# tontinton/dbeel

Measured on NVIDIA H100. Metric: compaction throughput MB/s (input bytes) at 1/2/4/8 H100 vs CPU shards, higher is better.
Workload: dtype u8

## Files before the change

dbeel_b200/csrc/dbeel_compact.cu:

```cuda
#include <cuda_runtime.h>
#include <math.h>
#include <stdint.h>
#include <stdio.h>
#include <stdlib.h>
#include <string.h>

#include <algorithm>
#include <atomic>
#include <deque>
#include <memory>
#include <new>
#include <thread>
#include <string>
#include <vector>

#include "../../include/dbeel_compact.h"
#include "kernels.cuh"
#include "merge_final.cuh"
#include "gather_async.cuh"
#include "gather_fb.cuh"
#include "gather_h.cuh"
#include "lookup.cuh"
#include "lookup_stream.cuh"
#include "route.cuh"
#include "scan.cuh"
#include "wal.cuh"
#include "host/scan_plan.h"
#include "host/stream_pump.h"

using namespace dbeel;

namespace {

constexpr uint64_t kAlign = 256;
inline uint64_t align_up(uint64_t v, uint64_t a) { return (v + a - 1) / a * a; }

enum { EV_START = 0, EV_EXTRACT, EV_MERGE, EV_RESOLVE, EV_GATHER, EV_H2D0, EV_H2D1, EV_D2H0, EV_D2H1, EV_COUNT };

}

struct dbeel_engine {
    int device = 0;
    cudaStream_t stream = nullptr;
    cudaEvent_t ev[EV_COUNT] = {};
    uint8_t *ws = nullptr;
    uint64_t ws_cap = 0;
    uint8_t *stage_in = nullptr, *stage_out = nullptr;
    uint64_t stage_in_cap = 0, stage_out_cap = 0;
    uint8_t *stage_in2 = nullptr, *stage_out2 = nullptr, *bloom_dev = nullptr;
    uint64_t stage_in2_cap = 0, stage_out2_cap = 0, bloom_dev_cap = 0;
    cudaStream_t s_h2d = nullptr, s_d2h = nullptr;
    cudaEvent_t ev_h2d[2] = {}, ev_comp[2] = {}, ev_d2h[2] = {};
    int pipeline = 1;
    uint64_t pipeline_min_bytes = 64ull << 20;
    uint64_t partition_bytes = 256ull << 20;
    int partition_taper = 1;
    uint8_t *ring_in = nullptr, *ring_out = nullptr, *pin_index = nullptr, *pin_bloom = nullptr;
    uint64_t ring_in_cap = 0, ring_out_cap = 0, pin_index_cap = 0, pin_bloom_cap = 0;
    int stream_ring = 3;
    uint8_t *wal_ws = nullptr;
    uint64_t wal_ws_cap = 0;
    uint8_t *route_ws = nullptr;
    uint64_t route_ws_cap = 0;
    uint8_t *pin = nullptr;
    uint8_t *pin_dev = nullptr;
    uint64_t pin_cap = 0;
    dbeel_stats stats = {};
    std::string err;
    bool busy = false;
    std::thread worker;
    std::atomic<int> async_state{0};
    int async_status = 0;
    std::vector<dbeel_run> async_runs;
    dbeel_compact_opts async_opts = {};
    uint8_t async_seed[32] = {};
    int sm_count = 0;
    int merge_variant = 1;
    int narrow_loads = 1;
    int gather_variant = 11;
    int fused_emit = 0;
    int bloom_side = 0;
    cudaStream_t s_side = nullptr;
    cudaEvent_t ev_fork = nullptr, ev_join = nullptr;
    int fused_final = 1;
    int fin_ctas_per_sm = 0;
    int pdl = 0;
    int stage_events = 1;
    int extract_persist = 6;
    int bloom_in_extract = 0;
};

namespace {

int fail(dbeel_engine *e, int code, const char *what, cudaError_t ce = cudaSuccess) {
    char buf[512];
    if (ce != cudaSuccess)
        snprintf(buf, sizeof buf, "%s: %s (%s)", what, cudaGetErrorName(ce), cudaGetErrorString(ce));
    else
        snprintf(buf, sizeof buf, "%s", what);
    if (e) e->err = buf;
    return code;
}

#define CU(call)                                                            \
    do {                                                                    \
        cudaError_t ce_ = (call);                                           \
        if (ce_ != cudaSuccess) return fail(e, DBEEL_ERR_CUDA, #call, ce_); \
    } while (0)

int ensure_device(dbeel_engine *e, uint8_t **buf, uint64_t *cap, uint64_t need) {
    if (need <= *cap) return DBEEL_OK;
    if (*buf) { cudaFree(*buf); *buf = nullptr; *cap = 0; }
    uint64_t want = align_up(need + need / 8, 1 << 20);
    cudaError_t ce = cudaMalloc(reinterpret_cast<void **>(buf), want);
    if (ce != cudaSuccess) {
        cudaGetLastError();
        want = align_up(need, 1 << 20);
        ce = cudaMalloc(reinterpret_cast<void **>(buf), want);
    }
    if (ce != cudaSuccess) { cudaGetLastError(); return fail(e, DBEEL_ERR_NOMEM, "cudaMalloc(workspace)", ce); }
    *cap = want;
    return DBEEL_OK;
}

int ensure_pinned(dbeel_engine *e, uint64_t need) {
    if (need <= e->pin_cap) return DBEEL_OK;
    if (e->pin) cudaFreeHost(e->pin);
    e->pin = nullptr;
    e->pin_dev = nullptr;
    e->pin_cap = 0;
    cudaError_t ce = cudaHostAlloc(reinterpret_cast<void **>(&e->pin), need, cudaHostAllocMapped);
    if (ce != cudaSuccess) { cudaGetLastError(); return fail(e, DBEEL_ERR_NOMEM, "cudaHostAlloc", ce); }
    ce = cudaHostGetDevicePointer(reinterpret_cast<void **>(&e->pin_dev), e->pin, 0);
    if (ce != cudaSuccess) { cudaGetLastError(); return fail(e, DBEEL_ERR_CUDA, "cudaHostGetDevicePointer", ce); }
    e->pin_cap = need;
    return DBEEL_OK;
}

int ensure_host(dbeel_engine *e, uint8_t **buf, uint64_t *cap, uint64_t need) {
    if (need <= *cap) return DBEEL_OK;
    if (*buf) { cudaFreeHost(*buf); *buf = nullptr; *cap = 0; }
    const uint64_t want = align_up(need + need / 8, 1 << 20);
    cudaError_t ce = cudaHostAlloc(reinterpret_cast<void **>(buf), want, cudaHostAllocDefault);
    if (ce != cudaSuccess) { cudaGetLastError(); *buf = nullptr; return fail(e, DBEEL_ERR_NOMEM, "cudaHostAlloc(stream ring)", ce); }
    *cap = want;
    return DBEEL_OK;
}

int stream_threads() {
    static const int n = [] {
        if (const char *v = getenv("DBEEL_IO_THREADS")) return std::max(1, atoi(v));
        const unsigned hw = std::thread::hardware_concurrency();
        return (int)std::min(8u, std::max(2u, hw / 8));
    }();
    return n;
}

template <class F>
int parallel_pieces(size_t n, F fn) {
    std::atomic<size_t> next{0};
    std::atomic<int> err{0};
    auto work = [&]() {
        for (size_t k = next.fetch_add(1); k < n && !err.load(); k = next.fetch_add(1)) {
            const int rc = fn(k);
            if (rc) { int z = 0; err.compare_exchange_strong(z, rc); }
        }
    };
    const int nt = (int)std::min<size_t>((size_t)stream_threads(), n);
// ... 274 lines not shown
            if (!f || fread(seed, 1, 32, f) != 32) {
                if (f) fclose(f);
                return fail(e, DBEEL_ERR_INVALID_ARG, "no entropy source for the bloom seed");
            }
            fclose(f);
        }
        p.bloom.words = reinterpret_cast<uint32_t *>(static_cast<uint8_t *>(out->bloom) + 8);
        p.bloom.bits = sh.bloom_bits;
        p.bloom.bits_magic = (uint64_t)((((unsigned __int128)1) << 64) / sh.bloom_bits);
        p.bloom.k_num = sh.bloom_k;
        for (int i = 0; i < 4; i++) memcpy(&p.bloom.sip[i], seed + 8 * i, 8);
    }
    if (extra) {
        p.sparse_offsets = extra->sparse_offsets ? 1 : 0;
        p.out_offset_base = extra->out_offset_base;
        if (extra->external_bloom) p.bloom = extra->bloom;
    }

    cudaStream_t s = e->stream;
    uint32_t launches = 0;
    if (record_start) CU(cudaEventRecord(e->ev[EV_START], s));
    launch_k(e, k_copy_words, (uint32_t)((header_bytes / 4 + 255) / 256), 256, 0, s, reinterpret_cast<uint32_t *>(ws),
             reinterpret_cast<const uint32_t *>(e->pin_dev), (uint32_t)(header_bytes / 4));
    launches++;
    if (sh.bloom_file) CU(cudaMemsetAsync(out->bloom, 0, sh.bloom_file, s));
    if (scan_bytes) CU(cudaMemsetAsync(ws + o_scan, 0, scan_bytes, s));

    const uint32_t g256 = (N + 255) / 256;
    const uint32_t gext = (N + 256 * kExtractEPT - 1) / (256 * kExtractEPT);
    auto launch_extract = [&](uint32_t grid, int mode) {
        if (ref_reader && hash_early) launch_k(e, k_extract<true, true, true>, grid, 256, 0, s, p, mode);
        else if (ref_reader) launch_k(e, k_extract<true, true, false>, grid, 256, 0, s, p, mode);
        else if (hash_early) launch_k(e, k_extract<true, false, true>, grid, 256, 0, s, p, mode);
        else if (e->narrow_loads && e->extract_persist > 0 && mode == 0)
            launch_k(e, k_extract<true, false, false, true>, std::min<uint32_t>(grid, (uint32_t)(e->sm_count * e->extract_persist)), 256, 0, s, p, mode);
        else if (e->narrow_loads) launch_k(e, k_extract<true, false, false>, grid, 256, 0, s, p, mode);
        else launch_k(e, k_extract<false, false, false>, grid, 256, 0, s, p, mode);
    };
    if (flush) {
        launch_k(e, k_flush_prefix_init, 1, 1, 0, s, p);
        launch_k(e, k_flush_prefix, g256, 256, 0, s, p);
        launch_extract(gext, 0);
        launch_k(e, k_plan, 1, 1024, 0, s, p);
        launch_k(e, k_block_sort, p.nseg[0], kMergeThreads, 0, s, p);
    } else {
        launch_k(e, k_common_prefix, 1, 32, 0, s, p, 0);
        launch_extract(gext, 0);
        if (ref_reader) {
            launch_k(e, k_ref_repair, n_runs, 1024, 0, s, p);
            launch_k(e, k_ref_reset, 1, 256, 0, s, p);
            launch_k(e, k_common_prefix, 1, 32, 0, s, p, 2);
            launch_extract(gext < 592 ? gext : 592, 2);
            launches += 4;
        }
        launch_k(e, k_common_prefix, 1, 32, 0, s, p, 1);
        launch_extract(gext < 592 ? gext : 592, 1);
        launch_k(e, k_plan, 1, 1024, 0, s, p);
    }
    launches += 5;
    if (!flush && (o->flags & DBEEL_FLAG_VERIFY_SORTED)) {
        launch_k(e, k_verify_sorted, g256, 256, 0, s, p);
        launches++;
    }
    const bool stage_ev = e->stage_events != 0;
    if (stage_ev) CU(cudaEventRecord(e->ev[EV_EXTRACT], s));

    const Rec *src = p.rec_a;
    Rec *dst = p.rec_b;
    if (sh.bloom_file) {
        launch_k(e, k_bloom_frame, 1, 1, 0, s, static_cast<uint8_t *>(out->bloom), sh.bloom_words, p.bloom);
        launches++;
    }
    for (uint32_t l = 0; l < levels; l++) {
        uint32_t pairs = p.nseg[l + 1];
        const bool last_fused = fused_final && l + 1 == levels;
        const uint64_t tl = last_fused ? kFinNominal : kMergeTile;
        uint64_t t_ub = (uint64_t)(N + tl - 1) / tl + pairs;
        uint64_t b_ub = t_ub + pairs;
        if (last_fused && stage_ev) CU(cudaEventRecord(e->ev[EV_MERGE], s));
        launch_k(e, k_merge_partition, (uint32_t)((b_ub + 7) / 8), kPartitionThreads, 0, s, p, l, src);
        if (last_fused) {
            uint64_t grid = (uint64_t)e->sm_count * e->fin_ctas_per_sm;
            if (grid > t_ub) grid = t_ub;
            if (e->narrow_loads) launch_k(e, k_merge_final<true>, (uint32_t)grid, kFinThreads, kFinSmem, s, p, l, src);
            else launch_k(e, k_merge_final<false>, (uint32_t)grid, kFinThreads, kFinSmem, s, p, l, src);
        } else if (e->merge_variant == 0) {
            launch_k(e, k_merge, (uint32_t)t_ub, kMergeThreads, 0, s, p, l, src, dst);
        } else {
            uint64_t grid = (uint64_t)e->sm_count * kMergeCtasPerSM;
            if (grid > t_ub) grid = t_ub;
            launch_k(e, k_merge_tma, (uint32_t)grid, kMergeThreads, 2 * kMergeBufRecs * sizeof(Rec), s, p, l, src, dst);
        }
        launches += 2;
        if (last_fused) break;
        const Rec *t = src;
        src = dst;
        dst = const_cast<Rec *>(t);
    }
    if (!fused_final && stage_ev) CU(cudaEventRecord(e->ev[EV_MERGE], s));

    if (jobs) {
        launch_k(e, k_bloom_frames, (extra->n_jobs + 127) / 128, 128, 0, s, p.groups, extra->n_jobs);
        launches++;
    }
    uint4 *res = reinterpret_cast<uint4 *>(dst);
    const bool side_bloom = e->bloom_side && !flush && !jobs && !hash_early && p.bloom.words != nullptr;
    p.bloom_elsewhere = side_bloom ? 1 : 0;
    if (!fused_final) {
        if (hash_early) launch_k(e, k_resolve<true, false, true>, (uint32_t)res_tiles, kResolveThreads, 0, s, p, src, res);
        else if (fused_emit) launch_k(e, k_resolve<true, true, false>, (uint32_t)res_tiles, kResolveThreads, 0, s, p, src, res);
        else if (e->narrow_loads) launch_k(e, k_resolve<true, false, false>, (uint32_t)res_tiles, kResolveThreads, 0, s, p, src, res);
        else launch_k(e, k_resolve<false, false, false>, (uint32_t)res_tiles, kResolveThreads, 0, s, p, src, res);
        launches += 1;
    }
    if (side_bloom) {
        CU(cudaEventRecord(e->ev_fork, s));
        CU(cudaStreamWaitEvent(e->s_side, e->ev_fork, 0));
        k_bloom_res<<<g256, 256, 0, e->s_side>>>(p, res);
        CU(cudaEventRecord(e->ev_join, e->s_side));
        launches++;
    }
    if (!fused_emit && !fused_final) {
        launch_k(e, k_scan_tiles, (uint32_t)res_chunks, 1024, 0, s, p);
        launch_k(e, k_scan_chunks, 1, 1024, 0, s, p);
        launch_k(e, k_emit, (uint32_t)res_tiles, kResolveThreads, 0, s, p, res);
        launches += 3;
    }
    if (n_groups) {
        launch_k(e, k_flush_table, (uint32_t)((n_groups + 1 + 127) / 128), 128, 0, s, p, res);
        launches++;
    }
    if (stage_ev) CU(cudaEventRecord(e->ev[EV_RESOLVE], s));

    if (gather_tiles) {
        const bool al32 = ((uintptr_t)out->data & 31) == 0;
        if (e->gather_variant == 11) {
            launch_k(e, k_gather_h, (uint32_t)gather_tiles, kGhThreads, 0, s, p);
        } else if (e->gather_variant == 2 && al32) {
            uint64_t grid = (uint64_t)e->sm_count * DBEEL_GT_CTAS;
            if (grid > gather_tiles) grid = gather_tiles;
            launch_k(e, k_gather_tma, (uint32_t)grid, kGtThreads, kGtSmem, s, p);
        } else if (e->gather_variant == 3 && al32) {
            uint64_t grid = (uint64_t)e->sm_count * DBEEL_GP_CTAS;
            if (grid > gather_tiles) grid = gather_tiles;
            launch_k(e, k_gather_p, (uint32_t)grid, kGatherThreads, 0, s, p);
        } else if (e->gather_variant == 4 && al32) {
            launch_k(e, k_gather32<true, false, false>, (uint32_t)gather_tiles, kGatherThreads + 32, 0, s, p);
        } else if (e->gather_variant == 8 && al32) {
            launch_k(e, k_gather_fb, (uint32_t)gather_tiles, kFbThreads, 0, s, p);
        } else if (e->gather_variant == 7 && al32) {
            launch_k(e, k_gather_async, (uint32_t)gather_tiles, kGatherThreads, 0, s, p);
        } else if (e->gather_variant >= 9 && al32) {
            launch_k(e, k_gather32<false, false, false, true>, (uint32_t)gather_tiles, kGatherThreads, 0, s, p);
        } else if (e->gather_variant == 5 && al32) {
            launch_k(e, k_gather32<false, true, false>, (uint32_t)gather_tiles, kGatherThreads, 0, s, p);
        } else if (e->gather_variant == 6 && al32 && p.bloom.words != nullptr && p.hash_rec == nullptr && !p.bloom_elsewhere &&
                   gather_tiles + (N + kGatherThreads - 1) / kGatherThreads < 0x7FFFFFFFull) {
            p.bloom_ctas = (uint32_t)((N + kGatherThreads - 1) / kGatherThreads);
            launch_k(e, k_gather32<false, false, true>, (uint32_t)(gather_tiles + p.bloom_ctas), kGatherThreads, 0, s, p);
        } else if (e->gather_variant >= 1 && al32) {
            launch_k(e, k_gather32<false, false, false>, (uint32_t)gather_tiles, kGatherThreads, 0, s, p);
        } else {
            launch_k(e, k_gather, (uint32_t)gather_tiles, kGatherThreads, 0, s, p);
        }
    }
    launches++;
    if (jobs) {
        launch_k(e, k_bloom_many, g256, 256, 0, s, p);
// ... 2067 lines not shown
            results[d].data_len += db;
            results[d].items_written += di;
        }
        out_bytes += bytes + 16 * items;
        pump.publish_pieces(c, std::move(pieces));
        if (c + 2 < np) rc = enqueue_h2d(c + 2);
    }
    if (rc) {
        cudaStreamSynchronize(e->s_h2d);
        cudaStreamSynchronize(s);
        cudaStreamSynchronize(e->s_d2h);
        pump.abort(rc);
        for (uint32_t d = 0; d < nd; d++) results[d] = dbeel_job_result{0, 0, 0, 0, 0, 0, 0};
        *stop = dbeel_scan_stop{-1, DBEEL_SCAN_STOP_NONE, 0};
        return rc;
    }
    CU(cudaEventRecord(e->ev[EV_GATHER], s));
    CU(cudaStreamSynchronize(s));
    CU(cudaStreamSynchronize(e->s_d2h));
    const int frc = pump.finish();
    if (frc) {
        for (uint32_t d = 0; d < nd; d++) results[d] = dbeel_job_result{0, 0, 0, 0, 0, 0, 0};
        *stop = dbeel_scan_stop{-1, DBEEL_SCAN_STOP_NONE, 0};
        return fail(e, frc, "stream write callback failed");
    }
    if (!stopped) host_stop();
    uint64_t items = 0;
    for (uint32_t d = 0; d < nd; d++) {
        results[d].index_len = 16 * results[d].items_written;
        items += results[d].items_written;
    }
    cudaEventElapsedTime(&e->stats.ms_total, e->ev[EV_START], e->ev[EV_GATHER]);
    e->stats.kernel_launches = launches + 1;
    e->stats.input_bytes = h2d_bytes;
    e->stats.output_bytes = out_bytes;
    e->stats.entries_out = items;
    return DBEEL_OK;
}

}


extern "C" {

int dbeel_abi_version(void) { return DBEEL_ABI_VERSION; }

int dbeel_engine_create(int device, dbeel_engine **out) {
    if (!out) return DBEEL_ERR_INVALID_ARG;
    *out = nullptr;
    int n = 0;
    if (cudaGetDeviceCount(&n) != cudaSuccess || n <= 0 || device < 0 || device >= n) {
        cudaGetLastError();
        return DBEEL_ERR_NO_DEVICE;
    }
    cudaDeviceProp prop;
    if (cudaGetDeviceProperties(&prop, device) != cudaSuccess) return DBEEL_ERR_CUDA;
    if (prop.major != 9 || prop.minor != 0) return DBEEL_ERR_NO_DEVICE;
    if (cudaSetDevice(device) != cudaSuccess) return DBEEL_ERR_CUDA;
    dbeel_engine *e = new (std::nothrow) dbeel_engine();
    if (!e) return DBEEL_ERR_NOMEM;
    e->device = device;
    e->sm_count = prop.multiProcessorCount;
    if (const char *v = getenv("DBEEL_MERGE")) e->merge_variant = atoi(v);
    if (const char *v = getenv("DBEEL_PIPELINE")) e->pipeline = atoi(v);
    if (const char *v = getenv("DBEEL_PIPELINE_MIN_KB")) e->pipeline_min_bytes = (uint64_t)(atoi(v) > 0 ? atoi(v) : 1) << 10;
    if (const char *v = getenv("DBEEL_PARTITION_KB")) e->partition_bytes = (uint64_t)(atoi(v) > 0 ? atoi(v) : 1) << 10;
    if (const char *v = getenv("DBEEL_PARTITION_TAPER")) e->partition_taper = atoi(v) != 0;
    if (const char *v = getenv("DBEEL_STREAM_RING")) e->stream_ring = std::max(2, atoi(v));
    if (const char *v = getenv("DBEEL_PARTITION_MB")) e->partition_bytes = (uint64_t)(atoi(v) > 0 ? atoi(v) : 128) << 20;
    if (cudaFuncSetAttribute(k_merge_tma, cudaFuncAttributeMaxDynamicSharedMemorySize, (int)(2 * kMergeBufRecs * sizeof(Rec))) != cudaSuccess ||
        cudaFuncSetAttribute(k_gather_tma, cudaFuncAttributeMaxDynamicSharedMemorySize, (int)kGtSmem) != cudaSuccess) {
        dbeel_engine_destroy(e);
        return DBEEL_ERR_CUDA;
    }
    if (const char *v = getenv("DBEEL_NARROW")) e->narrow_loads = atoi(v);
    if (const char *v = getenv("DBEEL_GATHER")) e->gather_variant = atoi(v);
    if (const char *v = getenv("DBEEL_BLOOM_EXTRACT")) e->bloom_in_extract = atoi(v);
    if (const char *v = getenv("DBEEL_BLOOM_SIDE")) e->bloom_side = atoi(v);
    if (const char *v = getenv("DBEEL_FUSED_EMIT")) e->fused_emit = atoi(v);
    if (const char *v = getenv("DBEEL_FUSED_FINAL")) e->fused_final = atoi(v);
    if (const char *v = getenv("DBEEL_EXTRACT_PERSIST")) e->extract_persist = atoi(v);
    if (const char *v = getenv("DBEEL_PDL")) e->pdl = atoi(v);
    if (const char *v = getenv("DBEEL_STAGE_EVENTS")) e->stage_events = atoi(v);
    {
        int nb_t = 0, nb_f = 0;
        if (cudaFuncSetAttribute(k_merge_final<true>, cudaFuncAttributeMaxDynamicSharedMemorySize, (int)kFinSmem) == cudaSuccess &&
            cudaFuncSetAttribute(k_merge_final<false>, cudaFuncAttributeMaxDynamicSharedMemorySize, (int)kFinSmem) == cudaSuccess &&
            cudaOccupancyMaxActiveBlocksPerMultiprocessor(&nb_t, k_merge_final<true>, kFinThreads, kFinSmem) == cudaSuccess &&
            cudaOccupancyMaxActiveBlocksPerMultiprocessor(&nb_f, k_merge_final<false>, kFinThreads, kFinSmem) == cudaSuccess) {
            e->fin_ctas_per_sm = std::min(std::min(nb_t, nb_f), (int)DBEEL_FIN_CTAS);
        } else {
            cudaGetLastError();
            e->fin_ctas_per_sm = 0;
        }
        if (const char *v = getenv("DBEEL_FIN_CTAS_RT")) e->fin_ctas_per_sm = std::min(e->fin_ctas_per_sm, std::max(1, atoi(v)));
    }
    if (cudaStreamCreateWithFlags(&e->s_side, cudaStreamNonBlocking) != cudaSuccess ||
        cudaEventCreateWithFlags(&e->ev_fork, cudaEventDisableTiming) != cudaSuccess ||
        cudaEventCreateWithFlags(&e->ev_join, cudaEventDisableTiming) != cudaSuccess) {
        dbeel_engine_destroy(e);
        return DBEEL_ERR_CUDA;
    }
    if (cudaStreamCreateWithFlags(&e->stream, cudaStreamNonBlocking) != cudaSuccess) { delete e; return DBEEL_ERR_CUDA; }
    for (int i = 0; i < EV_COUNT; i++)
        if (cudaEventCreate(&e->ev[i]) != cudaSuccess) { dbeel_engine_destroy(e); return DBEEL_ERR_CUDA; }
    *out = e;
    return DBEEL_OK;
}

void *dbeel_engine_stream(dbeel_engine *e) { return e ? static_cast<void *>(e->stream) : nullptr; }

void dbeel_engine_destroy(dbeel_engine *e) {
    if (!e) return;
    if (e->worker.joinable()) e->worker.join();
    cudaSetDevice(e->device);
    if (e->stream) cudaStreamSynchronize(e->stream);
    for (int i = 0; i < EV_COUNT; i++)
        if (e->ev[i]) cudaEventDestroy(e->ev[i]);
    if (e->ws) cudaFree(e->ws);
    if (e->stage_in) cudaFree(e->stage_in);
    if (e->stage_out) cudaFree(e->stage_out);
    if (e->stage_in2) cudaFree(e->stage_in2);
    if (e->stage_out2) cudaFree(e->stage_out2);
    if (e->bloom_dev) cudaFree(e->bloom_dev);
    if (e->wal_ws) cudaFree(e->wal_ws);
    if (e->route_ws) cudaFree(e->route_ws);
    for (int i = 0; i < 2; i++) {
        if (e->ev_h2d[i]) cudaEventDestroy(e->ev_h2d[i]);
        if (e->ev_comp[i]) cudaEventDestroy(e->ev_comp[i]);
        if (e->ev_d2h[i]) cudaEventDestroy(e->ev_d2h[i]);
    }
    if (e->ev_fork) cudaEventDestroy(e->ev_fork);
    if (e->ev_join) cudaEventDestroy(e->ev_join);
    if (e->s_side) cudaStreamDestroy(e->s_side);
    if (e->s_h2d) cudaStreamDestroy(e->s_h2d);
    if (e->s_d2h) cudaStreamDestroy(e->s_d2h);
    if (e->pin) cudaFreeHost(e->pin);
    if (e->ring_in) cudaFreeHost(e->ring_in);
    if (e->ring_out) cudaFreeHost(e->ring_out);
    if (e->pin_index) cudaFreeHost(e->pin_index);
    if (e->pin_bloom) cudaFreeHost(e->pin_bloom);
    if (e->stream) cudaStreamDestroy(e->stream);
    delete e;
}

uint64_t dbeel_bloom_bitmap_bytes(uint64_t items, double fp) {
    const double ln2 = 0.693147180559945309417232121458176568;
    return (uint64_t)ceil((double)items * log(fp) / (-8.0 * (ln2 * ln2)));
}

uint32_t dbeel_bloom_k_num(uint64_t bitmap_bits, uint64_t items) {
    uint32_t k = (uint32_t)ceil((double)bitmap_bits / (double)items * log(2.0));
    return k < 1 ? 1 : k;
}

uint64_t dbeel_bloom_file_size(uint64_t items, double fp) {
    uint64_t bits = dbeel_bloom_bitmap_bytes(items, fp) * 8;
    return 8 + 4 * ((bits + 31) / 32) + 8 + 8 + 4 + 144;
}

int dbeel_compact_bound(const dbeel_run *runs, uint32_t n_runs, const dbeel_compact_opts *opts, uint64_t *data_cap,
                        uint64_t *index_cap, uint64_t *bloom_cap) {
    if (n_runs && !runs) return DBEEL_ERR_INVALID_ARG;
    dbeel_compact_opts o;
    default_opts(&o);
    if (opts) o = *opts;
    if (!(o.bloom_fp > 0.0 && o.bloom_fp < 1.0)) return DBEEL_ERR_INVALID_ARG;
    JobShape sh;
    shape_of(runs, n_runs, &o, false, &sh);
    if (data_cap) *data_cap = sh.data_total;
    if (index_cap) *index_cap = sh.n_total * 16;
    if (bloom_cap) *bloom_cap = sh.bloom_file;
    return DBEEL_OK;
}

#define REFUSE_WHILE_ASYNC(e)                                                                  \
// ... 293 lines not shown
```

dbeel_b200/csrc/merge_final.cuh:

```cuda
#pragma once
#include "kernels.cuh"

namespace dbeel {

constexpr int kFinThreads = kMergeThreads;
constexpr int kFinVT = kMergeVT;
constexpr int kFinTile = kMergeTile;
constexpr int kFinNominal = kFinTile - 64;
constexpr int kFinBufRecs = kFinTile + 8;
constexpr int kFinMaxRunsSmem = 64;
#ifndef DBEEL_FIN_CTAS
#define DBEEL_FIN_CTAS 2
#endif
constexpr uint32_t kFinSmem = 2u * kFinBufRecs * 16u + 2u * kFinTile * 8u + (uint32_t)kFinTile + 16u;

#ifdef DBEEL_FIN_PHASES
constexpr int kFinPhases = 8;
__device__ unsigned long long g_fin_phase[kFinPhases];
__device__ unsigned int g_fin_done;
#define FIN_PH_DECL unsigned long long ph_acc[kFinPhases] = {}; long long ph_t = clock64();
#define FIN_PH(k) do { if (tid == 0) { const long long ph_n = clock64(); ph_acc[k] += (unsigned long long)(ph_n - ph_t); ph_t = ph_n; } } while (0)
__device__ __forceinline__ void fin_phase_flush(const unsigned long long *acc, uint32_t n_tiles) {
    for (int k = 0; k < kFinPhases; k++) atomicAdd(&g_fin_phase[k], acc[k]);
    __threadfence();
    if (atomicAdd(&g_fin_done, 1u) + 1 == (gridDim.x < n_tiles ? gridDim.x : n_tiles)) {
        __threadfence();
        unsigned long long v[kFinPhases], tot = 0;
        for (int k = 0; k < kFinPhases; k++) { v[k] = atomicExch(&g_fin_phase[k], 0ull); tot += v[k]; }
        g_fin_done = 0;
        printf("fin_phases ctas=%u cycles=%llu tma=%llu merge=%llu index_issue=%llu index_wait=%llu lookback=%llu emit=%llu "
               "ts_wait=%llu heads_scan=%llu\n", gridDim.x, tot, v[0], v[1], v[2], v[3], v[4], v[5], v[6], v[7]);
    }
}
#else
#define FIN_PH_DECL
#define FIN_PH(k) do {} while (0)
#endif

struct FinDesc {
    uint32_t a_src, n_a, b_src, n_b;
    uint32_t a_end, b_end;
    uint32_t diag0;
    uint32_t nb;
};

__device__ __forceinline__ void fin_lookback(const unsigned long long *scan_state, uint32_t t, uint32_t lane, unsigned long long &eb,
                                             uint32_t &ec) {
    constexpr int kPer = 4;
    eb = 0;
    ec = 0;
    for (int base = (int)t - 1;; base -= 32 * kPer) {
        unsigned long long vb[kPer], vc[kPer];
#pragma unroll
        for (int k = 0; k < kPer; k++) {
            const int idx = base - (int)lane * kPer - k;
            vb[k] = kScanPrefix << 62;
            vc[k] = kScanPrefix << 32;
            if (idx >= 0) {
                vc[k] = ld_volatile_u64(scan_state + 2ull * (uint32_t)idx + 1);
                vb[k] = ld_volatile_u64(scan_state + 2ull * (uint32_t)idx);
            }
        }
        bool found = false;
        unsigned long long sb = 0;
        uint32_t sc = 0;
#pragma unroll
        for (int k = 0; k < kPer; k++) {
            const int idx = base - (int)lane * kPer - k;
            while ((vc[k] >> 32) == 0 || (vc[k] >> 32) != (vb[k] >> 62)) {
                vc[k] = ld_volatile_u64(scan_state + 2ull * (uint32_t)idx + 1);
                vb[k] = ld_volatile_u64(scan_state + 2ull * (uint32_t)idx);
            }
            if (!found) {
                sb += vb[k] & ((1ull << 62) - 1);
                sc += (uint32_t)vc[k];
                found = (vc[k] >> 32) == kScanPrefix;
            }
        }
        const uint32_t fm = __ballot_sync(0xFFFFFFFFu, found);
        const uint32_t first = fm ? (uint32_t)__ffs((int)fm) - 1u : 32u;
        if (lane > first) { sb = 0; sc = 0; }
#pragma unroll
        for (int o = 16; o; o >>= 1) {
            sb += __shfl_xor_sync(0xFFFFFFFFu, sb, o);
            sc += __shfl_xor_sync(0xFFFFFFFFu, sc, o);
        }
        eb += sb;
        ec += sc;
        if (fm) return;
    }
}

template <bool kNarrow>
__global__ void __launch_bounds__(kFinThreads, DBEEL_FIN_CTAS) k_merge_final(const __grid_constant__ Params p, uint32_t level, const Rec *src) {
    constexpr int NT = kFinThreads, VT = kFinVT;
    extern __shared__ __align__(128) uint8_t f_raw[];
    Rec *bufs[2] = {reinterpret_cast<Rec *>(f_raw), reinterpret_cast<Rec *>(f_raw) + kFinBufRecs};
    unsigned long long *s_tlo = reinterpret_cast<unsigned long long *>(f_raw + 2u * kFinBufRecs * 16u);
    unsigned long long *s_thi = s_tlo + kFinTile;
    uint8_t *s_flag = reinterpret_cast<uint8_t *>(s_thi + kFinTile);
    __shared__ __align__(8) uint64_t s_bar[2];
    __shared__ Rec s_bnd[5];
    __shared__ unsigned long long s_wb[NT / 32];
    __shared__ uint32_t s_wc[NT / 32];
    __shared__ unsigned long long s_pref[2];
    __shared__ uint32_t s_rbase[kFinMaxRunsSmem + 1];
    __shared__ uint8_t s_rlut[256];
    __shared__ const uint4 *s_rindex[kFinMaxRunsSmem];
    __shared__ const uint8_t *s_rdata[kFinMaxRunsSmem];

    pdl_trigger();
    pdl_wait();
    const uint32_t tid = threadIdx.x, lane = tid & 31, warp = tid >> 5;
    const uint32_t skip = p.ctl->prefix_len + kWindowBytes;
    const uint32_t n_tiles = p.tile_base[level][p.nseg[level + 1]];
    const uint32_t G = gridDim.x;
    uint32_t tile = blockIdx.x;
    if (tile >= n_tiles) return;
    const bool runs_cached = p.n_runs <= (uint32_t)kFinMaxRunsSmem;
    uint32_t lut_shift = 0;
    while (((uint64_t)p.n_total >> lut_shift) > 256) lut_shift++;
    if (runs_cached) {
        for (uint32_t r = tid; r < p.n_runs; r += NT) {
            s_rbase[r] = p.runs[r].base;
            s_rindex[r] = p.runs[r].index;
            s_rdata[r] = p.runs[r].data;
        }
        if (tid == 0) s_rbase[p.n_runs] = 0xFFFFFFFFu;
        s_rlut[tid] = (uint8_t)find_run(p, (uint32_t)(((uint64_t)tid << lut_shift) < p.n_total ? (uint64_t)tid << lut_shift : p.n_total - 1));
    }
    if (tid == 0) {
        mbar_init(&s_bar[0], 1);
        mbar_init(&s_bar[1], 1);
        s_pref[0] = s_pref[1] = ~0ull;
        asm volatile("fence.mbarrier_init.release.cluster;" ::: "memory");
    }
    __syncthreads();
    FIN_PH_DECL

    auto run_of = [&](uint32_t gid) -> uint32_t {
        if (!runs_cached) return find_run(p, gid);
        uint32_t r = s_rlut[gid >> lut_shift];
        while (s_rbase[r + 1] <= gid) r++;
        return r;
    };
    auto index_ptr = [&](uint32_t gid, uint32_t r) -> const uint4 * {
        return runs_cached ? s_rindex[r] + (gid - s_rbase[r]) : p.runs[r].index + (gid - p.runs[r].base);
    };
    auto data_ptr = [&](uint32_t r) -> const uint8_t * { return runs_cached ? s_rdata[r] : p.runs[r].data; };

    auto issue = [&](const FinDesc &d, Rec *buf, uint64_t *bar) {
        const uint32_t ap = d.nb & 1u, an = (d.nb >> 1) & 1u, bp = (d.nb >> 2) & 1u, bn = (d.nb >> 3) & 1u;
        const uint32_t ca = d.n_a + ap + an, cb = d.n_b + bp + bn;
        asm volatile("fence.proxy.async.shared::cta;" ::: "memory");
        mbar_expect_tx(bar, (ca + cb) * 16u);
        if (ca) tma_load_1d(buf + 1 - ap, &src[d.a_src - ap], ca * 16u, bar);
        if (cb) tma_load_1d(buf + d.n_a + 3 - bp, &src[d.b_src - bp], cb * 16u, bar);
    };

    const Seg segA = p.seg[level][0];
    Seg segB;
    segB.start = 0; segB.len = 0;
    if (p.nseg[level] > 1) segB = p.seg[level][1];
    auto ld_bidx = [&](uint32_t t) -> uint32_t { return t < n_tiles ? __ldg(&p.tile_bnd[t]) : 0xFFFFFFFFu; };
    auto mk_desc = [&](uint32_t bidx) -> FinDesc {
        FinDesc d;
        d.a_src = d.n_a = d.b_src = d.n_b = d.a_end = d.b_end = d.diag0 = d.nb = 0;
        if (bidx == 0xFFFFFFFFu) return d;
        const uint4 b0 = __ldg(&p.bnd[bidx]), b1 = __ldg(&p.bnd[bidx + 1]);
        d.a_src = b0.x; d.n_a = b1.x - b0.x;
        d.b_src = b0.y; d.n_b = b1.y - b0.y;
        d.a_end = segA.start + segA.len;
        d.b_end = segB.start + segB.len;
        d.diag0 = b0.z;
        d.nb = (b0.x > segA.start ? 1u : 0u) | (b1.x < d.a_end ? 2u : 0u) | (b0.y > segB.start ? 4u : 0u) | (b1.y < d.b_end ? 8u : 0u);
        return d;
    };
    FinDesc cur = mk_desc(ld_bidx(tile));
    FinDesc nxt = mk_desc(ld_bidx(tile + G));
    uint32_t bidx2 = ld_bidx(tile + 2 * G);
    if (tid == 0) issue(cur, bufs[0], &s_bar[0]);
    const int keep_tombstones = p.keep_tombstones;

    uint32_t prev_tile = 0, prev_d = 0, prev_act = 0, prev_pos = 0, prev_tc = 0;
    unsigned long long prev_off = 0, prev_tb = 0;
    volatile unsigned long long *vpref = s_pref;
    auto finish_prev = [&](uint32_t prev_q) {
        const unsigned long long tag = prev_q & 0xFFFFu;
        if (warp == 0) {
            unsigned long long eb = 0;
            uint32_t ec = 0;
            if (prev_tile > 0) fin_lookback(p.scan_state, prev_tile, lane, eb, ec);
            if (lane == 0) {
                if (prev_tile > 0) {
                    unsigned long long *mine = p.scan_state + 2ull * prev_tile;
                    st_volatile_u64(mine, (kScanPrefix << 62) | (eb + prev_tb));
                    st_volatile_u64(mine + 1, (kScanPrefix << 32) | (unsigned long long)(ec + prev_tc));
                }
                vpref[0] = (tag << 48) | eb;
                vpref[1] = (tag << 32) | ec;
                if (prev_tile + 1 == n_tiles) {
                    Ctl *cw = p.ctl;
                    cw->out_data_len = eb + prev_tb;
                    cw->out_items = ec + prev_tc;
                }
            }
        }
        unsigned long long pb, pc;
        do {
            pb = vpref[0];
            pc = vpref[1];
        } while ((pb >> 48) != tag || (pc >> 32) != tag);
        FIN_PH(4);
        unsigned long long off = (pb & ((1ull << 48) - 1)) + prev_off;
        uint32_t pos = (uint32_t)pc + prev_pos;
        constexpr unsigned long long gt = kGatherTileBytes;
#pragma unroll
        for (int i = 0; i < VT; i++) {
            if (!((prev_act >> i) & 1u)) continue;
            const unsigned long long sz = s_thi[prev_d + i];
            const uint32_t fs = (uint32_t)(sz >> 32);
            if (!fs) continue;
            const unsigned long long file_off = off + p.out_offset_base;
            p.out_index[pos] = make_uint4((uint32_t)file_off, (uint32_t)(file_off >> 32), (uint32_t)sz, fs);
            p.src_ptr[pos] = s_tlo[prev_d + i];
            for (unsigned long long bq = (off + gt - 1) / gt; bq * gt < off + fs && bq < p.tile_first_n; bq++) p.tile_first[bq] = pos;
            off += fs;
            pos++;
        }
        FIN_PH(5);
    };

    uint32_t q = 0;
    for (;; q++) {
        Rec *s = bufs[q & 1];
        uint4 *s4 = reinterpret_cast<uint4 *>(s);
        const bool has_next = tile + G < n_tiles;
        if (tid == 0 && has_next) issue(nxt, bufs[(q + 1) & 1], &s_bar[(q + 1) & 1]);
        const FinDesc nn = mk_desc(bidx2);
        const uint32_t bidx3 = ld_bidx(tile + 3 * G);
        while (!mbar_try_wait(&s_bar[q & 1], (q >> 1) & 1)) {}
        FIN_PH(0);

        const uint32_t nA = cur.n_a, nB = cur.n_b, n = nA + nB;
        const Rec *A = s + 1, *B = s + nA + 3;
        uint32_t d = tid * VT;
        if (d > n) d = n;
        Rec me[VT + 1];
        {
            uint32_t lo = d > nB ? d - nB : 0;
            uint32_t hi = d < nA ? d : nA;
            while (lo < hi) {
                const uint32_t mid = (lo + hi) >> 1;
                if (!key_less_smem(p, skip, &B[d - 1 - mid], &A[mid])) lo = mid + 1; else hi = mid;
            }
            uint32_t ai = lo, bi = d - lo;
            Rec ak = A[ai], bk = B[bi];
#pragma unroll
            for (int i = 0; i < VT; i++) {
                const bool has_a = ai < nA, has_b = bi < nB;
                const bool take_b = has_b && (!has_a || key_less(p, skip, bk, ak));
                me[i] = take_b ? bk : ak;
                if (take_b) { bi++; bk = B[bi]; } else { ai++; ak = A[ai]; }
            }
            if (tid == 0) {
                s_bnd[0] = s[0];
                s_bnd[1] = s[nA + 1];
                s_bnd[2] = s[nA + 2];
                s_bnd[3] = s[nA + 3 + nB];
            }
            __syncthreads();
            if (d < n) s[d] = me[0];
            if (d + VT - 1 < n) s[d + VT - 1] = me[VT - 1];
#pragma unroll
            for (int i = 0; i < VT; i++)
                if (d + i == n - 1) s_bnd[4] = me[i];
        }
        __syncthreads();
        FIN_PH(1);

        uint32_t m_act = 0, m_eqn = 0, m_eqp = 0;
        uint32_t gidv[VT];
        uint4 irec[VT];
        {
#pragma unroll
            for (int i = 0; i < VT; i++)
                if (d + i < n) m_act |= 1u << i;
            me[VT].x = me[VT].y = me[VT].z = me[VT].w = 0;
            if (d + VT < n) me[VT] = s[d + VT];
#pragma unroll
            for (int i = 0; i < VT; i++) {
                if (!(m_act & (1u << i))) continue;
                bool eqn;
                if (d + i + 1 < n) {
                    eqn = key_equal(p, skip, me[i], me[i + 1]);
                } else {
                    eqn = ((cur.nb & 2u) && key_equal(p, skip, me[i], s_bnd[1])) || ((cur.nb & 8u) && key_equal(p, skip, me[i], s_bnd[3]));
                }
                if (eqn) m_eqn |= 1u << i;
            }
            m_eqp = m_eqn << 1;
            if (m_act & 1u) {
                bool eqp;
                if (d > 0) eqp = key_equal(p, skip, s[d - 1], me[0]);
                else eqp = ((cur.nb & 1u) && key_equal(p, skip, s_bnd[0], me[0])) || ((cur.nb & 4u) && key_equal(p, skip, s_bnd[2], me[0]));
                if (eqp) m_eqp |= 1u;
            }
#pragma unroll
            for (int i = 0; i < VT; i++) {
                gidv[i] = me[i].w;
                irec[i] = make_uint4(0, 0, 0, 0);
                if (m_act & (1u << i)) {
                    const uint32_t r = run_of(gidv[i]);
                    const uint4 *q4 = index_ptr(gidv[i], r);
                    irec[i] = kNarrow ? ldg128_narrow(q4) : __ldg(q4);
                }
            }
        }
        __syncthreads();
        FIN_PH(2);
        {
            const uint32_t m_grp = m_act & (m_eqn | m_eqp);
            unsigned long long tlo[VT], thi[VT];
#pragma unroll
            for (int i = 0; i < VT; i++) {
                tlo[i] = thi[i] = 0;
                if (!(m_act & (1u << i))) continue;
                const uint32_t r = run_of(gidv[i]);
                const uint8_t *entry = data_ptr(r) + ((uint64_t)irec[i].x | ((uint64_t)irec[i].y << 32));
                const unsigned long long ea = (unsigned long long)(uintptr_t)entry;
                s4[d + i] = make_uint4((uint32_t)ea, (uint32_t)(ea >> 32), irec[i].z, irec[i].w);
                if ((m_grp >> i) & 1u) {
                    const uint8_t *t = entry + irec[i].w - 16;
                    if (kNarrow) { tlo[i] = ld_u64_unaligned_narrow(t); thi[i] = ld_u64_unaligned_narrow(t + 8); }
                    else { tlo[i] = ld_u64_unaligned(t); thi[i] = ld_u64_unaligned(t + 8); }
                    s_flag[d + i] = (uint8_t)((m_eqn >> i) & 1u);
                }
            }
            FIN_PH(3);
            if (q > 0) finish_prev(q - 1);
#pragma unroll
            for (int i = 0; i < VT; i++) {
                if ((m_grp >> i) & 1u) { s_tlo[d + i] = tlo[i]; s_thi[d + i] = thi[i]; }
            }
        }
        __syncthreads();
        FIN_PH(6);

        unsigned long long vb = 0;
        uint32_t vc = 0;
        uint4 we[VT];
#pragma unroll
        for (int i = 0; i < VT; i++) {
            we[i] = make_uint4(0, 0, 0, 0);
            if (!((m_act >> i) & 1u) || ((m_eqp >> i) & 1u)) continue;
            const uint32_t k = d + i;
            uint4 info = s4[k];
            if ((m_eqn >> i) & 1u) {
                unsigned long long wlo = s_tlo[k], whi = s_thi[k];
                uint32_t j = k;
                bool more = true;
                while (more && j + 1 < n) {
                    j++;
                    const unsigned long long clo = s_tlo[j], chi = s_thi[j];
                    if (!ts_greater(wlo, whi, clo, chi)) { info = s4[j]; wlo = clo; whi = chi; }
                    more = s_flag[j] != 0;
                }
                if (more) {
                    const Rec last = s_bnd[4];
                    for (int side = 0; side < 2; side++) {
                        uint32_t g = side ? cur.b_src + nB : cur.a_src + nA;
                        const uint32_t end = side ? cur.b_end : cur.a_end;
                        for (; g < end; g++) {
                            const Rec nx = ld_rec(&src[g]);
                            if (!key_equal(p, skip, last, nx)) break;
                            const KeyRef ck = key_of_gid(p, nx.w);
                            uint64_t clo, chi;
                            ld_ts(ck.entry, ck.full_size, &clo, &chi);
                            if (!ts_greater(wlo, whi, clo, chi)) {
                                const unsigned long long ea = (unsigned long long)(uintptr_t)ck.entry;
                                info = make_uint4((uint32_t)ea, (uint32_t)(ea >> 32), ck.klen + 8, ck.full_size);
                                wlo = clo; whi = chi;
                            }
                        }
                    }
                }
            }
            const bool tomb = info.w == info.z + 24;
            if (keep_tombstones || !tomb) {
                we[i] = info;
                vb += info.w;
                vc += 1;
            }
        }

        unsigned long long ib = vb;
        uint32_t ic = vc;
#pragma unroll
        for (int o = 1; o < 32; o <<= 1) {
            const unsigned long long xb = __shfl_up_sync(0xFFFFFFFFu, ib, o);
            const uint32_t xc = __shfl_up_sync(0xFFFFFFFFu, ic, o);
            if (lane >= (uint32_t)o) { ib += xb; ic += xc; }
        }
        if (lane == 31) { s_wb[warp] = ib; s_wc[warp] = ic; }
        __syncthreads();
        unsigned long long tb = 0, wbefore = 0;
        uint32_t tc = 0, wcbefore = 0;
#pragma unroll
        for (int w = 0; w < NT / 32; w++) {
            if ((uint32_t)w < warp) { wbefore += s_wb[w]; wcbefore += s_wc[w]; }
            tb += s_wb[w];
            tc += s_wc[w];
        }
        if (tid == 0) {
            const unsigned long long st = tile == 0 ? kScanPrefix : kScanAgg;
            unsigned long long *mine = p.scan_state + 2ull * tile;
            st_volatile_u64(mine, (st << 62) | tb);
            st_volatile_u64(mine + 1, (st << 32) | tc);
        }
#pragma unroll
        for (int i = 0; i < VT; i++) {
            if ((m_act >> i) & 1u) {
                s_tlo[d + i] = (unsigned long long)we[i].x | ((unsigned long long)we[i].y << 32);
                s_thi[d + i] = (unsigned long long)we[i].z | ((unsigned long long)we[i].w << 32);
            }
        }
        prev_tile = tile;
        prev_d = d;
        prev_act = m_act;
        prev_off = wbefore + ib - vb;
        prev_pos = wcbefore + ic - vc;
        prev_tb = tb;
        prev_tc = tc;
        if (!has_next) {
            FIN_PH(7);
            break;
        }
        asm volatile("fence.proxy.async.shared::cta;" ::: "memory");
        __syncthreads();
        FIN_PH(7);
        tile += G;
        cur = nxt;
        nxt = nn;
        bidx2 = bidx3;
    }
    finish_prev(q);
#ifdef DBEEL_FIN_PHASES
    if (tid == 0) fin_phase_flush(ph_acc, n_tiles);
#endif
}

}
```

Baseline: 813,300.

## Prefetch final-merge index records into shared memory via cp.async

Adds a prefetch variant of the fused final merge kernel, on by default. It gathers each tile's index records into the spare shared buffer with cp.async ahead of time, replacing per-thread global index loads after the merge. The timestamp loads become aligned 64-bit loads with shift-based realignment, and the decoupled lookback uses a smaller per-lane window. The trade-off is that the next tile's TMA load can only start once the spare buffer is free again, which reduces overlap of bulk loads with compute and adds extra barriers.

```diff
diff --git a/dbeel_b200/csrc/dbeel_compact.cu b/dbeel_b200/csrc/dbeel_compact.cu
--- a/dbeel_b200/csrc/dbeel_compact.cu
+++ b/dbeel_b200/csrc/dbeel_compact.cu
@@ -84,6 +84,7 @@
     cudaEvent_t ev_fork = nullptr, ev_join = nullptr;
     int fused_final = 1;
     int fin_ctas_per_sm = 0;
+    int fin_prefetch = 1;
     int pdl = 0;
     int stage_events = 1;
     int extract_persist = 6;
@@ -524,8 +525,9 @@
         if (last_fused) {
             uint64_t grid = (uint64_t)e->sm_count * e->fin_ctas_per_sm;
             if (grid > t_ub) grid = t_ub;
-            if (e->narrow_loads) launch_k(e, k_merge_final<true>, (uint32_t)grid, kFinThreads, kFinSmem, s, p, l, src);
-            else launch_k(e, k_merge_final<false>, (uint32_t)grid, kFinThreads, kFinSmem, s, p, l, src);
+            auto kfin = e->narrow_loads ? (e->fin_prefetch ? k_merge_final<true, true> : k_merge_final<true, false>)
+                                        : (e->fin_prefetch ? k_merge_final<false, true> : k_merge_final<false, false>);
+            launch_k(e, kfin, (uint32_t)grid, kFinThreads, kFinSmem, s, p, l, src);
         } else if (e->merge_variant == 0) {
             launch_k(e, k_merge, (uint32_t)t_ub, kMergeThreads, 0, s, p, l, src, dst);
         } else {
@@ -2759,16 +2761,17 @@
     if (const char *v = getenv("DBEEL_EXTRACT_PERSIST")) e->extract_persist = atoi(v);
     if (const char *v = getenv("DBEEL_PDL")) e->pdl = atoi(v);
     if (const char *v = getenv("DBEEL_STAGE_EVENTS")) e->stage_events = atoi(v);
+    if (const char *v = getenv("DBEEL_FIN_PREFETCH")) e->fin_prefetch = atoi(v);
     {
-        int nb_t = 0, nb_f = 0;
-        if (cudaFuncSetAttribute(k_merge_final<true>, cudaFuncAttributeMaxDynamicSharedMemorySize, (int)kFinSmem) == cudaSuccess &&
-            cudaFuncSetAttribute(k_merge_final<false>, cudaFuncAttributeMaxDynamicSharedMemorySize, (int)kFinSmem) == cudaSuccess &&
-            cudaOccupancyMaxActiveBlocksPerMultiprocessor(&nb_t, k_merge_final<true>, kFinThreads, kFinSmem) == cudaSuccess &&
-            cudaOccupancyMaxActiveBlocksPerMultiprocessor(&nb_f, k_merge_final<false>, kFinThreads, kFinSmem) == cudaSuccess) {
-            e->fin_ctas_per_sm = std::min(std::min(nb_t, nb_f), (int)DBEEL_FIN_CTAS);
-        } else {
-            cudaGetLastError();
-            e->fin_ctas_per_sm = 0;
+        e->fin_ctas_per_sm = (int)DBEEL_FIN_CTAS;
+        for (auto kfin : {k_merge_final<true, true>, k_merge_final<true, false>, k_merge_final<false, true>, k_merge_final<false, false>}) {
+            int nb = 0;
+            if (cudaFuncSetAttribute(kfin, cudaFuncAttributeMaxDynamicSharedMemorySize, (int)kFinSmem) != cudaSuccess ||
+                cudaOccupancyMaxActiveBlocksPerMultiprocessor(&nb, kfin, kFinThreads, kFinSmem) != cudaSuccess) {
+                cudaGetLastError();
+                nb = 0;
+            }
+            e->fin_ctas_per_sm = std::min(e->fin_ctas_per_sm, nb);
         }
         if (const char *v = getenv("DBEEL_FIN_CTAS_RT")) e->fin_ctas_per_sm = std::min(e->fin_ctas_per_sm, std::max(1, atoi(v)));
     }
diff --git a/dbeel_b200/csrc/merge_final.cuh b/dbeel_b200/csrc/merge_final.cuh
--- a/dbeel_b200/csrc/merge_final.cuh
+++ b/dbeel_b200/csrc/merge_final.cuh
@@ -17,24 +17,29 @@
 #ifdef DBEEL_FIN_PHASES
 constexpr int kFinPhases = 8;
 __device__ unsigned long long g_fin_phase[kFinPhases];
+__device__ unsigned long long g_fin_count[3];
 __device__ unsigned int g_fin_done;
-#define FIN_PH_DECL unsigned long long ph_acc[kFinPhases] = {}; long long ph_t = clock64();
+#define FIN_PH_DECL unsigned long long ph_acc[kFinPhases] = {}, cnt_acc[3] = {}; long long ph_t = clock64();
 #define FIN_PH(k) do { if (tid == 0) { const long long ph_n = clock64(); ph_acc[k] += (unsigned long long)(ph_n - ph_t); ph_t = ph_n; } } while (0)
+#define FIN_CNT(k, v) (cnt_acc[k] += (v))
 __device__ __forceinline__ void fin_phase_flush(const unsigned long long *acc, uint32_t n_tiles) {
     for (int k = 0; k < kFinPhases; k++) atomicAdd(&g_fin_phase[k], acc[k]);
     __threadfence();
     if (atomicAdd(&g_fin_done, 1u) + 1 == (gridDim.x < n_tiles ? gridDim.x : n_tiles)) {
         __threadfence();
-        unsigned long long v[kFinPhases], tot = 0;
+        unsigned long long v[kFinPhases], c[3], tot = 0;
         for (int k = 0; k < kFinPhases; k++) { v[k] = atomicExch(&g_fin_phase[k], 0ull); tot += v[k]; }
+        for (int k = 0; k < 3; k++) c[k] = atomicExch(&g_fin_count[k], 0ull);
         g_fin_done = 0;
         printf("fin_phases ctas=%u cycles=%llu tma=%llu merge=%llu index_issue=%llu index_wait=%llu lookback=%llu emit=%llu "
-               "ts_wait=%llu heads_scan=%llu\n", gridDim.x, tot, v[0], v[1], v[2], v[3], v[4], v[5], v[6], v[7]);
+               "ts_wait=%llu heads_scan=%llu records=%llu ts_loads=%llu survivors=%llu\n", gridDim.x, tot, v[0], v[1], v[2], v[3],
+               v[4], v[5], v[6], v[7], c[0], c[1], c[2]);
     }
 }
 #else
 #define FIN_PH_DECL
 #define FIN_PH(k) do {} while (0)
+#define FIN_CNT(k, v) do {} while (0)
 #endif
 
 struct FinDesc {
@@ -46,7 +51,7 @@
 
 __device__ __forceinline__ void fin_lookback(const unsigned long long *scan_state, uint32_t t, uint32_t lane, unsigned long long &eb,
                                              uint32_t &ec) {
-    constexpr int kPer = 4;
+    constexpr int kPer = 2;
     eb = 0;
     ec = 0;
     for (int base = (int)t - 1;; base -= 32 * kPer) {
@@ -92,6 +97,14 @@
 }
 
 template <bool kNarrow>
+__device__ __forceinline__ uint64_t fin_ldg64(const uint64_t *q) {
+    if (!kNarrow) return __ldg(q);
+    uint64_t v;
+    asm("ld.global.nc.L2::64B.u64 %0, [%1];" : "=l"(v) : "l"(q));
+    return v;
+}
+
+template <bool kNarrow, bool kPrefetch>
 __global__ void __launch_bounds__(kFinThreads, DBEEL_FIN_CTAS) k_merge_final(const __grid_constant__ Params p, uint32_t level, const Rec *src) {
     constexpr int NT = kFinThreads, VT = kFinVT;
     extern __shared__ __align__(128) uint8_t f_raw[];
@@ -148,6 +161,17 @@
         return runs_cached ? s_rindex[r] + (gid - s_rbase[r]) : p.runs[r].index + (gid - p.runs[r].base);
     };
     auto data_ptr = [&](uint32_t r) -> const uint8_t * { return runs_cached ? s_rdata[r] : p.runs[r].data; };
+
+    auto prefetch_index = [&](const FinDesc &d, const Rec *buf, Rec *slots) {
+        for (uint32_t k = tid; k < d.n_a + d.n_b; k += NT) {
+            const uint32_t pos = k < d.n_a ? 1 + k : 3 + k;
+            const uint32_t gid = buf[pos].w;
+            const uint4 *q4 = index_ptr(gid, run_of(gid));
+            if (kNarrow) asm volatile("cp.async.cg.shared.global.L2::64B [%0], [%1], 16;" ::"r"(smem_u32(&slots[pos])), "l"(q4) : "memory");
+            else cp_async16(&slots[pos], q4);
+        }
+        asm volatile("cp.async.commit_group;" ::: "memory");
+    };
 
     auto issue = [&](const FinDesc &d, Rec *buf, uint64_t *bar) {
         const uint32_t ap = d.nb & 1u, an = (d.nb >> 1) & 1u, bp = (d.nb >> 2) & 1u, bn = (d.nb >> 3) & 1u;
@@ -180,6 +204,10 @@
     FinDesc nxt = mk_desc(ld_bidx(tile + G));
     uint32_t bidx2 = ld_bidx(tile + 2 * G);
     if (tid == 0) issue(cur, bufs[0], &s_bar[0]);
+    if (kPrefetch) {
+        while (!mbar_try_wait(&s_bar[0], 0)) {}
+        prefetch_index(cur, bufs[0], bufs[1]);
+    }
     const int keep_tombstones = p.keep_tombstones;
 
     uint32_t prev_tile = 0, prev_d = 0, prev_act = 0, prev_pos = 0, prev_tc = 0;
@@ -234,12 +262,13 @@
     uint32_t q = 0;
     for (;; q++) {
         Rec *s = bufs[q & 1];
+        Rec *other = bufs[(q + 1) & 1];
         uint4 *s4 = reinterpret_cast<uint4 *>(s);
         const bool has_next = tile + G < n_tiles;
-        if (tid == 0 && has_next) issue(nxt, bufs[(q + 1) & 1], &s_bar[(q + 1) & 1]);
+        if (!kPrefetch && tid == 0 && has_next) issue(nxt, other, &s_bar[(q + 1) & 1]);
         const FinDesc nn = mk_desc(bidx2);
         const uint32_t bidx3 = ld_bidx(tile + 3 * G);
-        while (!mbar_try_wait(&s_bar[q & 1], (q >> 1) & 1)) {}
+        if (!kPrefetch) while (!mbar_try_wait(&s_bar[q & 1], (q >> 1) & 1)) {}
         FIN_PH(0);
 
         const uint32_t nA = cur.n_a, nB = cur.n_b, n = nA + nB;
@@ -247,6 +276,7 @@
         uint32_t d = tid * VT;
         if (d > n) d = n;
         Rec me[VT + 1];
+        uint32_t srcp[VT];
         {
             uint32_t lo = d > nB ? d - nB : 0;
             uint32_t hi = d < nA ? d : nA;
@@ -261,6 +291,7 @@
                 const bool has_a = ai < nA, has_b = bi < nB;
                 const bool take_b = has_b && (!has_a || key_less(p, skip, bk, ak));
                 me[i] = take_b ? bk : ak;
+                srcp[i] = take_b ? nA + 3 + bi : 1 + ai;
                 if (take_b) { bi++; bk = B[bi]; } else { ai++; ak = A[ai]; }
             }
             if (tid == 0) {
@@ -310,21 +341,38 @@
             for (int i = 0; i < VT; i++) {
                 gidv[i] = me[i].w;
                 irec[i] = make_uint4(0, 0, 0, 0);
-                if (m_act & (1u << i)) {
+                if (!kPrefetch && (m_act & (1u << i))) {
                     const uint32_t r = run_of(gidv[i]);
                     const uint4 *q4 = index_ptr(gidv[i], r);
                     irec[i] = kNarrow ? ldg128_narrow(q4) : __ldg(q4);
                 }
             }
         }
+        if (kPrefetch) {
+            FIN_PH(2);
+            asm volatile("cp.async.wait_all;" ::: "memory");
+        }
         __syncthreads();
-        FIN_PH(2);
+        if (kPrefetch) {
+            const uint4 *o4 = reinterpret_cast<const uint4 *>(other);
+#pragma unroll
+            for (int i = 0; i < VT; i++)
+                if (m_act & (1u << i)) irec[i] = o4[srcp[i]];
+            asm volatile("fence.proxy.async.shared::cta;" ::: "memory");
+            __syncthreads();
+            if (tid == 0 && has_next) issue(nxt, other, &s_bar[(q + 1) & 1]);
+        } else {
+            FIN_PH(2);
+        }
         {
             const uint32_t m_grp = m_act & (m_eqn | m_eqp);
-            unsigned long long tlo[VT], thi[VT];
+            FIN_CNT(0, __popc(m_act));
+            FIN_CNT(1, __popc(m_grp));
+            unsigned long long tlo[VT], thi[VT], tx[VT];
+            uint32_t tsh = 0;
 #pragma unroll
             for (int i = 0; i < VT; i++) {
-                tlo[i] = thi[i] = 0;
+                tlo[i] = thi[i] = tx[i] = 0;
                 if (!(m_act & (1u << i))) continue;
                 const uint32_t r = run_of(gidv[i]);
                 const uint8_t *entry = data_ptr(r) + ((uint64_t)irec[i].x | ((uint64_t)irec[i].y << 32));
@@ -332,8 +380,18 @@
                 s4[d + i] = make_uint4((uint32_t)ea, (uint32_t)(ea >> 32), irec[i].z, irec[i].w);
                 if ((m_grp >> i) & 1u) {
                     const uint8_t *t = entry + irec[i].w - 16;
-                    if (kNarrow) { tlo[i] = ld_u64_unaligned_narrow(t); thi[i] = ld_u64_unaligned_narrow(t + 8); }
-                    else { tlo[i] = ld_u64_unaligned(t); thi[i] = ld_u64_unaligned(t + 8); }
+                    if (kPrefetch) {
+                        const uintptr_t ta = reinterpret_cast<uintptr_t>(t);
+                        const uint64_t *a = reinterpret_cast<const uint64_t *>(ta & ~uintptr_t(7));
+                        tsh |= (uint32_t)(ta & 7) << (3 * i);
+                        tlo[i] = fin_ldg64<kNarrow>(a);
+                        thi[i] = fin_ldg64<kNarrow>(a + 1);
+                        if (ta & 7) tx[i] = fin_ldg64<kNarrow>(a + 2);
+                    } else if (kNarrow) {
+                        tlo[i] = ld_u64_unaligned_narrow(t); thi[i] = ld_u64_unaligned_narrow(t + 8);
+                    } else {
+                        tlo[i] = ld_u64_unaligned(t); thi[i] = ld_u64_unaligned(t + 8);
+                    }
                     s_flag[d + i] = (uint8_t)((m_eqn >> i) & 1u);
                 }
             }
@@ -341,7 +399,15 @@
             if (q > 0) finish_prev(q - 1);
 #pragma unroll
             for (int i = 0; i < VT; i++) {
-                if ((m_grp >> i) & 1u) { s_tlo[d + i] = tlo[i]; s_thi[d + i] = thi[i]; }
+                if (!((m_grp >> i) & 1u)) continue;
+                unsigned long long lo = tlo[i], hi = thi[i];
+                const uint32_t sh = ((tsh >> (3 * i)) & 7u) * 8u;
+                if (kPrefetch && sh) {
+                    lo = (tlo[i] >> sh) | (thi[i] << (64 - sh));
+                    hi = (thi[i] >> sh) | (tx[i] << (64 - sh));
+                }
+                s_tlo[d + i] = lo;
+                s_thi[d + i] = hi;
             }
         }
         __syncthreads();
@@ -394,6 +460,7 @@
             }
         }
 
+        FIN_CNT(2, vc);
         unsigned long long ib = vb;
         uint32_t ic = vc;
 #pragma unroll
@@ -424,6 +491,13 @@
                 s_tlo[d + i] = (unsigned long long)we[i].x | ((unsigned long long)we[i].y << 32);
                 s_thi[d + i] = (unsigned long long)we[i].z | ((unsigned long long)we[i].w << 32);
             }
+        }
+        if (kPrefetch && has_next) {
+            FIN_PH(7);
+            while (!mbar_try_wait(&s_bar[(q + 1) & 1], ((q + 1) >> 1) & 1)) {}
+            FIN_PH(0);
+            prefetch_index(nxt, other, s);
+            FIN_PH(2);
         }
         prev_tile = tile;
         prev_d = d;
@@ -446,6 +520,8 @@
     }
     finish_prev(q);
 #ifdef DBEEL_FIN_PHASES
+    for (int k = 0; k < 3; k++) atomicAdd(&g_fin_count[k], cnt_acc[k]);
+    __syncthreads();
     if (tid == 0) fin_phase_flush(ph_acc, n_tiles);
 #endif
 }
```

After: 834,200 (median of 6 runs). 1.03x the previous value.
